# mahbhlddnhakkh/yuv-manipulations-2

Hardware: AMD Instinct MI355X
Metric: megapixels/sec DCT compress+decompress, 4K IYUV; achieved HBM GB/s vs peak (higher is better)
Workload: dtype u8/int16 (fp32 transform)

## Files before the change

yuv-manipulations-2_amd/csrc/fdct_bfly.h:

```cpp
#pragma once

#if defined(__HIPCC__)
#define MYYUV_BF_HD __host__ __device__ __forceinline__
#else
#include <math.h>
#define MYYUV_BF_HD static inline
#endif

namespace myyuv_bfly {

constexpr float kC0 = 0.3535533845424652f, kC4 = 0.3535534143447876f;
constexpr float kA2 = 0.4619397521018982f, kB2 = 0.19134166836738586f;
constexpr float kA6 = 0.4619397521018982f, kB6 = 0.19134169816970825f;
constexpr float kO1[4] = {0.49039262533187866f, 0.41573476791381836f, 0.27778512239456177f, 0.09754513204097748f};
constexpr float kO3[4] = {0.41573482751846313f, -0.0975450873374939f, -0.49039262533187866f, -0.277785062789917f};
constexpr float kO5[4] = {0.2777852416038513f, -0.49039262533187866f, 0.09754514694213867f, 0.41573476791381836f};
constexpr float kO7[4] = {0.09754543751478195f, -0.2777852416038513f, 0.4157347083091736f, -0.49039262533187866f};
constexpr float kBflyK = 7.946e-7f;

MYYUV_BF_HD float odd4(const float (&o)[4], float d0, float d1, float d2, float d3) {
  return fmaf(o[3], d3, fmaf(o[2], d2, fmaf(o[1], d1, o[0] * d0)));
}

MYYUV_BF_HD void bfly_cols(const float (&p)[8], float (&t)[8]) {
  const float s0 = p[0] + p[7], s1 = p[1] + p[6], s2 = p[2] + p[5], s3 = p[3] + p[4];
  const float d0 = p[0] - p[7], d1 = p[1] - p[6], d2 = p[2] - p[5], d3 = p[3] - p[4];
  const float ss0 = s0 + s3, ss1 = s1 + s2, ds0 = s0 - s3, ds1 = s1 - s2;
  t[0] = kC0 * ((ss0 + ss1) - 1024.0f);
  t[4] = kC4 * (ss0 - ss1);
  t[2] = fmaf(kA2, ds0, kB2 * ds1);
  t[6] = fmaf(kB6, ds0, -kA6 * ds1);
  t[1] = odd4(kO1, d0, d1, d2, d3);
  t[3] = odd4(kO3, d0, d1, d2, d3);
  t[5] = odd4(kO5, d0, d1, d2, d3);
  t[7] = odd4(kO7, d0, d1, d2, d3);
}

MYYUV_BF_HD void bfly_rows(const float (&x)[8], float (&y)[8]) {
  const float s0 = x[0] + x[7], s1 = x[1] + x[6], s2 = x[2] + x[5], s3 = x[3] + x[4];
  const float d0 = x[0] - x[7], d1 = x[1] - x[6], d2 = x[2] - x[5], d3 = x[3] - x[4];
  const float ss0 = s0 + s3, ss1 = s1 + s2, ds0 = s0 - s3, ds1 = s1 - s2;
  y[0] = kC0 * (ss0 + ss1);
  y[4] = kC4 * (ss0 - ss1);
  y[2] = fmaf(kA2, ds0, kB2 * ds1);
  y[6] = fmaf(kB6, ds0, -kA6 * ds1);
  y[1] = odd4(kO1, d0, d1, d2, d3);
  y[3] = odd4(kO3, d0, d1, d2, d3);
  y[5] = odd4(kO5, d0, d1, d2, d3);
  y[7] = odd4(kO7, d0, d1, d2, d3);
}

MYYUV_BF_HD void bfly_row_bounds(const float* r, float* kb) {
  for (int i = 0; i < 8; i++) {
    double m = 0.0;
    for (int v = 0; v < 8; v++) m = r[i * 8 + v] > m ? r[i * 8 + v] : m;
    kb[i] = (float)((double)kBflyK * m * (1.0 + 0x1p-20) * (1.0 + 0x1p-22));
  }
}

#if !defined(__HIPCC__)
static inline int bfly_block(const unsigned char* px, const float* R, const float* kb, short* out) {
  unsigned a = 0;
  for (int i = 0; i < 64; i++) a += px[i] > 128 ? px[i] - 128u : 128u - px[i];
  const float af = (float)a;
  float T[8][8];
  for (int k = 0; k < 8; k++) {
    float p[8], t[8];
    for (int m = 0; m < 8; m++) p[m] = (float)px[m * 8 + k];
    bfly_cols(p, t);
    for (int i = 0; i < 8; i++) T[i][k] = t[i];
  }
  int ok = 1;
  for (int i = 0; i < 8; i++) {
    float y[8];
    bfly_rows(T[i], y);
    float em = 0.0f;
    for (int v = 0; v < 8; v++) {
      const float t = y[v] * R[i * 8 + v];
      const float uu = t + 0x1.8p23f;
      const float e = t - (uu - 0x1.8p23f);
      em = fmaxf(em, fabsf(e));
      out[i * 8 + v] = (short)(int)(uu - 0x1.8p23f);
    }
    if (fmaf(af, kb[i], em) >= 0.5f) ok = 0;
// ... 7 lines not shown
```

yuv-manipulations-2_amd/csrc/k_transform.hip:

```cpp
#include <stddef.h>

#include "codec_common.hpp"
#include "xform_common.hpp"

#ifndef MYYUV_K1_OCC
#define MYYUV_K1_OCC 8
#endif
#define MYYUV_K1_ATTR __attribute__((amdgpu_waves_per_eu(MYYUV_K1_OCC, MYYUV_K1_OCC)))

namespace myyuv_gpu {

using namespace xf;

typedef unsigned short k1_us2 __attribute__((ext_vector_type(2)));

__device__ __forceinline__ void store_block_rows(const uint32_t (&c)[16], uint32_t q, uint32_t lane, bool live,
                                                 uint32_t g, uint4* dlo, uint4* dhi, uint8_t* __restrict__ rmask,
                                                 uint32_t* __restrict__ binfo, const uint4* zq,
                                                 uint4* __restrict__ sink) {
  uint4 lo, hi;
  uint32_t rm;
  pack_quads(c, q, lo, hi, rm);
  const uint4 z0 = zq[0], z1 = zq[1];
  const uint32_t wv[8] = {lo.x, lo.y, lo.z, lo.w, hi.x, hi.y, hi.z, hi.w};
  const uint32_t zv[8] = {z0.x, z0.y, z0.z, z0.w, z1.x, z1.y, z1.z, z1.w};
  k1_us2 cnt = {0, 0}, mx = {0, 0};
#pragma unroll
  for (int i = 0; i < 8; i++) {
    uint32_t fu, m16;
    asm("v_pk_min_u16 %0, %1, %2" : "=v"(fu) : "v"(wv[i]), "s"(0x00010001u));
    cnt += __builtin_bit_cast(k1_us2, fu);
    asm("v_pk_mul_lo_u16 %0, %1, %2" : "=v"(m16) : "v"(fu), "v"(zv[i]));
    mx = __builtin_elementwise_max(mx, __builtin_bit_cast(k1_us2, m16));
  }
  uint32_t nnz = (uint32_t)cnt.x + (uint32_t)cnt.y;
  uint32_t msz = mx.x > mx.y ? (uint32_t)mx.x : (uint32_t)mx.y;
#pragma unroll
  for (int d = 1; d < 4; d <<= 1) {
    const uint32_t o = d == 1 ? quad_xor1(nnz | (msz << 16)) : quad_xor2(nnz | (msz << 16));
    nnz += o & 0xFFFFu;
    msz = max(msz, o >> 16);
  }
  const bool nzl = (rm >> (2 * q)) & 1u, nzh = (rm >> (2 * q + 1)) & 1u;
  *(live ? rmask + g : reinterpret_cast<uint8_t*>(sink + 128) + lane) = (uint8_t)rm;
  const uint32_t dc = quad_lane0(lo.x);
  *(live ? binfo + g : reinterpret_cast<uint32_t*>(sink + 132) + lane) = binfo_word(rm, msz, class_of(nnz, msz), dc);
  *(nzl ? dlo : sink + lane) = lo;
  *(nzh ? dhi : sink + 64 + lane) = hi;
}

#ifndef MYYUV_K1_BUF
#define MYYUV_K1_BUF 1
#endif
typedef unsigned int k1_v4u __attribute__((ext_vector_type(4)));
constexpr uint32_t kOob = 0xFFFFFFFFu;

struct K1Rsrc {
  __amdgpu_buffer_rsrc_t coef, rmask, binfo;
};
__device__ __forceinline__ K1Rsrc k1_rsrc(uint4* coef, uint8_t* rmask, uint32_t* binfo, const FrameGeom& G) {
  const uint32_t nblk = G.cum[3] * G.nframes;
  K1Rsrc r;
  r.coef = __builtin_amdgcn_make_buffer_rsrc(coef, 0, (int)(((nblk + 63u) / 64u) * (kCoefQuadsPerWave * 16u)),
                                             0x00020000);
  r.rmask = __builtin_amdgcn_make_buffer_rsrc(rmask, 0, (int)nblk, 0x00020000);
  r.binfo = __builtin_amdgcn_make_buffer_rsrc(binfo, 0, (int)(nblk * 4u), 0x00020000);
  return r;
}

__device__ __forceinline__ void store_block_rows_buf(const uint32_t (&c)[16], uint32_t q, bool live, uint32_t g,
                                                     const K1Rsrc& R, const uint4* zq) {
  uint4 lo, hi;
  uint32_t rm;
  pack_quads(c, q, lo, hi, rm);
  const uint4 z0 = zq[0], z1 = zq[1];
  const uint32_t wv[8] = {lo.x, lo.y, lo.z, lo.w, hi.x, hi.y, hi.z, hi.w};
  const uint32_t zv[8] = {z0.x, z0.y, z0.z, z0.w, z1.x, z1.y, z1.z, z1.w};
  k1_us2 cnt = {0, 0}, mx = {0, 0};
#pragma unroll
  for (int i = 0; i < 8; i++) {
    uint32_t fu, m16;
    asm("v_pk_min_u16 %0, %1, %2" : "=v"(fu) : "v"(wv[i]), "s"(0x00010001u));
    cnt += __builtin_bit_cast(k1_us2, fu);
    asm("v_pk_mul_lo_u16 %0, %1, %2" : "=v"(m16) : "v"(fu), "v"(zv[i]));
    mx = __builtin_elementwise_max(mx, __builtin_bit_cast(k1_us2, m16));
  }
  uint32_t nnz = (uint32_t)cnt.x + (uint32_t)cnt.y;
  uint32_t msz = mx.x > mx.y ? (uint32_t)mx.x : (uint32_t)mx.y;
#pragma unroll
  for (int d = 1; d < 4; d <<= 1) {
    const uint32_t o = d == 1 ? quad_xor1(nnz | (msz << 16)) : quad_xor2(nnz | (msz << 16));
    nnz += o & 0xFFFFu;
    msz = max(msz, o >> 16);
  }
  const bool nzl = (rm >> (2 * q)) & 1u, nzh = (rm >> (2 * q + 1)) & 1u;
  const uint32_t dc = quad_lane0(lo.x);
  __builtin_amdgcn_raw_buffer_store_b8((uint8_t)rm, R.rmask, live ? g : kOob, 0, 0);
  __builtin_amdgcn_raw_buffer_store_b32(binfo_word(rm, msz, class_of(nnz, msz), dc), R.binfo, live ? 4u * g : kOob,
                                        0, 0);
  const uint32_t qo = coef_quad(g, 2 * q) * 16u;
  __builtin_amdgcn_raw_buffer_store_b128(k1_v4u{lo.x, lo.y, lo.z, lo.w}, R.coef, live && nzl ? qo : kOob, 0, 0);
  __builtin_amdgcn_raw_buffer_store_b128(k1_v4u{hi.x, hi.y, hi.z, hi.w}, R.coef, live && nzh ? qo + 1024u : kOob, 0,
                                         0);
}

__device__ __forceinline__ void stage_zz(uint4* szz) {
  if (threadIdx.x < 32) reinterpret_cast<uint32_t*>(szz)[threadIdx.x] = kZzPairs.v[threadIdx.x];
}


__global__ __launch_bounds__(256) MYYUV_K1_ATTR void k_fdct_quant(const uint8_t* __restrict__ frame, FrameGeom G,
                                                   const QTables* __restrict__ qt,
                                                   uint4* __restrict__ coef, uint8_t* __restrict__ rmask,
                                                   uint32_t* __restrict__ binfo, uint4* __restrict__ sink,
                                                   uint32_t* __restrict__ k2ctl, uint32_t* __restrict__ fix,
                                                   uint32_t par) {
  if (k2ctl != nullptr && blockIdx.x == 0 && threadIdx.x == 0) *k2ctl = 0u;
  __shared__ float tile[4][kXfUnit * kTile];
  __shared__ float sqr[kSqWords];
  __shared__ uint4 szz[8];
  static_assert(offsetof(QTables, r) == sizeof(float) * kSqR && offsetof(QTables, kb) == sizeof(float) * kSqKb,
                "layout");
  stage_zz(szz);
  stage_tables<kSqWords>(qt->q[0], sqr);
  if (kSinkSlots > 1) sink += (size_t)((blockIdx.x * 4u + (threadIdx.x >> 6)) % kSinkSlots) * kSinkQuads;
  const uint32_t lane = threadIdx.x & 63u;
  const uint32_t q = lane & 3u, b = lane >> 2;
  float* tb = tile[threadIdx.x >> 6] + b * kTile;
  uint8_t* img = reinterpret_cast<uint8_t*>(tb);
#if MYYUV_K1_BUF
  const K1Rsrc rs = k1_rsrc(coef, rmask, binfo, G);
#endif
  const uint32_t nall = G.ucum[3] * G.nframes, stride = unit_stride();
  uint32_t ua = first_unit();
  uint4 nx = ua < nall ? load_rows(frame, G, ua, b, q) : make_uint4(0, 0, 0, 0);
  sink[lane] = make_uint4(0, 0, 0, 0);
  sink[64 + lane] = make_uint4(0, 0, 0, 0);
  reinterpret_cast<uint8_t*>(sink + 128)[lane] = 0;

  for (; ua < nall; ua += stride) {
    const uint32_t f = div_magic(ua, G.umag);
    const Unit U = unit_of(G, ua - f * G.ucum[3]);
    const uint32_t local = U.local0 + b;
    const bool live = local < U.nb;
    const uint32_t g = f * G.cum[3] + U.cum + local;
    *reinterpret_cast<uint2*>(img + 16u * q) = make_uint2(nx.x, nx.y);
    *reinterpret_cast<uint2*>(img + 16u * q + 8u) = make_uint2(nx.z, nx.w);
    nx = load_rows(frame, G, ua + stride < nall ? ua + stride : ua, b, q);
    wave_sync();

    auto store = [&](const uint32_t (&c)[16], bool keep) {
      const bool lv = live && keep;
#if MYYUV_K1_BUF
      store_block_rows_buf(c, q, lv, g, rs, szz + 2 * q);
#else
      uint4* dlo = lv ? coef + coef_quad(g, 2 * q) : sink + lane;
      uint4* dhi = lv ? coef + coef_quad(g, 2 * q + 1) : sink + 64 + lane;
      store_block_rows(c, q, lane, lv, g, dlo, dhi, rmask, binfo, szz + 2 * q, sink);
#endif
    };
    uint32_t xr[4];
    fdct_load(img, q, xr);
    const uint64_t bad = fdct_fast<true>(xr, tb, q, sqr, U.p, store);
    if (bad != 0) {
      const bool mine = ((bad >> lane) & 1u) && q == 0 && live;
      const uint64_t m = __ballot(mine);
      const uint32_t c = ua % kFixLists;
      uint32_t base = 0;
      if (lane == 0 && m != 0) base = atomicAdd(fix_count(fix, par, c), (uint32_t)__popcll(m));
      base = __builtin_amdgcn_readfirstlane(base);
      const uint32_t idx = base + __builtin_amdgcn_mbcnt_hi((uint32_t)(m >> 32), __builtin_amdgcn_mbcnt_lo((uint32_t)m, 0u));
      if (mine && idx < fix_list_cap(nall)) fix_list(fix, G, c)[idx] = ua * kXfUnit + b;
    }
  }
}

__global__ __launch_bounds__(64 * kFixWaves) void k_fdct_fix(const uint8_t* __restrict__ frame, FrameGeom G,
                                                  const QTables* __restrict__ qt, uint4* __restrict__ coef,
                                                  uint8_t* __restrict__ rmask, uint32_t* __restrict__ binfo,
                                                  uint4* __restrict__ sink,
                                                  uint32_t* __restrict__ fix, uint32_t par) {
  __shared__ float tile[kFixWaves][kXfUnit * kTile];
  __shared__ float sqr[2 * 3 * 64];
  __shared__ uint4 szz[8];
  __shared__ uint32_t s_any;
  if (blockIdx.x == 0 && threadIdx.x < kFixLists) *fix_count(fix, par ^ 1u, threadIdx.x) = 0u;
  if (threadIdx.x == 0) s_any = 0u;
  __syncthreads();
  const uint32_t gw = blockIdx.x * kFixWaves + (threadIdx.x >> 6), nw = gridDim.x * kFixWaves;
  const uint32_t c = gw % kFixLists;
  const uint32_t n = __builtin_amdgcn_readfirstlane(*fix_count(fix, par, c));
  if ((threadIdx.x & 63u) == 0 && gw / kFixLists * kXfUnit < n) s_any = 1u;
  __syncthreads();
  if (s_any == 0u) return;
  stage_zz(szz);
#pragma unroll
  for (uint32_t i = threadIdx.x; i < 2u * 3u * 64u; i += 64u * kFixWaves) sqr[i] = qt->q[0][i];
  __syncthreads();
  const uint32_t lane = threadIdx.x & 63u;
  const uint32_t q = lane & 3u, b = lane >> 2;
  float* tb = tile[threadIdx.x >> 6] + b * kTile;
  uint8_t* img = reinterpret_cast<uint8_t*>(tb);
  const uint32_t* list = fix_list(fix, G, c);
#if MYYUV_K1_BUF
  const K1Rsrc rs = k1_rsrc(coef, rmask, binfo, G);
#endif
  for (uint32_t i = gw / kFixLists * kXfUnit; i < n; i += nw / kFixLists * kXfUnit) {
    const bool real = i + b < n;
    const uint32_t ent = list[real ? i + b : i];
    const uint32_t ua = ent / kXfUnit, bb = ent % kXfUnit;
    const uint32_t f = div_magic(ua, G.umag);
    const Unit U = unit_of(G, ua - f * G.ucum[3]);
    const uint32_t g = f * G.cum[3] + U.cum + U.local0 + bb;
    const uint4 r = load_rows(frame, G, ua, bb, q);
    wave_sync();
    *reinterpret_cast<uint2*>(img + 16u * q) = make_uint2(r.x, r.y);
    *reinterpret_cast<uint2*>(img + 16u * q + 8u) = make_uint2(r.z, r.w);
    wave_sync();
    uint32_t xr[4];
    fdct_load(img, q, xr);
#if MYYUV_K1_BUF
    fdct_exact(xr, tb, q, sqr, U.p, [&](const uint32_t (&cc)[16]) { store_block_rows_buf(cc, q, real, g, rs, szz + 2 * q); });
#else
    uint4* dlo = real ? coef + coef_quad(g, 2 * q) : sink + lane;
    uint4* dhi = real ? coef + coef_quad(g, 2 * q + 1) : sink + 64 + lane;
    fdct_exact(xr, tb, q, sqr, U.p,
               [&](const uint32_t (&cc)[16]) {
                 store_block_rows(cc, q, lane, real, g, dlo, dhi, rmask, binfo, szz + 2 * q, sink);
               });
#endif
  }
}

__global__ __launch_bounds__(256) void k_dequant_idct(const uint4* __restrict__ coef,
                                                     const uint8_t* __restrict__ rmask,
                                                     const uint4* __restrict__ zq, FrameGeom G,
                                                     const QTables* __restrict__ qt,
                                                     uint8_t* __restrict__ frame, uint4* __restrict__ sink) {
  __shared__ float tile[4][kXfUnit * kTile];
  __shared__ float sq[3 * 64];
  stage_tables<3 * 64>(qt->q[0], sq);
  const uint32_t lane = threadIdx.x & 63u;
  const uint32_t q = lane & 3u, b = lane >> 2;
// ... 102 lines not shown
```

yuv-manipulations-2_amd/csrc/myyuv_hip.cpp:

```cpp
#include <hip/hip_ext.h>
#include <hip/hip_runtime.h>

#include <algorithm>
#include <cmath>
#include <cstdio>
#include <cstdlib>
#include <cstring>
#include <mutex>
#include <vector>

#include "codec_common.hpp"
#include "fdct_bfly.h"
#include "k_chain.hpp"
#include "k_stream.hpp"
#include "myyuv_hip.h"

#ifndef MYYUV_R16_BATCH
#define MYYUV_R16_BATCH 1
#endif

namespace myyuv_gpu {
__global__ void k_fdct_quant(const uint8_t*, FrameGeom, const QTables*, uint4*, uint8_t*, uint32_t*, uint4*,
                             uint32_t*, uint32_t*, uint32_t);
__global__ void k_fdct_fix(const uint8_t*, FrameGeom, const QTables*, uint4*, uint8_t*, uint32_t*, uint4*,
// ... 1243 lines not shown
  std::vector<uint8_t> rm(n);
  if (hipStreamSynchronize(c->stream) != hipSuccess ||
      hipMemcpy(img.data(), c->coef.p, nq * 16, hipMemcpyDeviceToHost) != hipSuccess ||
      hipMemcpy(rm.data(), c->rmask.p, n, hipMemcpyDeviceToHost) != hipSuccess)
    return MYYUV_E_HIP;
  for (uint32_t b = 0; b < n; b++)
    for (uint32_t q = 0; q < 8; q++) {
      if ((rm[b] >> q) & 1u)
        std::memcpy(out + (size_t)b * 64 + q * 8, &img[coef_quad(b, q)], 16);
      else
        std::memset(out + (size_t)b * 64 + q * 8, 0, 16);
    }
  return 0;
}

int myyuv_debug_tinfo_guard(myyuv_hip_handle c, uint32_t ntiles, int arm, uint32_t* changed) {
  if (!c) return MYYUV_E_ARG;
  std::lock_guard<std::mutex> lk(c->mu);
  DeviceGuard g(c->device);
  constexpr uint32_t kGuardWords = kWinTilesBig * kTInfoWords;
  constexpr uint32_t kCanary = 0xA5C3E1F7u;
  const size_t off = (size_t)ntiles * kTInfoWords * 4;
  if (off + kGuardWords * 4 > c->tinfo.n) return MYYUV_E_ARG;
  std::vector<uint32_t> w(kGuardWords, kCanary);
  if (hipStreamSynchronize(c->stream) != hipSuccess) return MYYUV_E_HIP;
  uint8_t* p = static_cast<uint8_t*>(c->tinfo.p) + off;
  if (arm) return hipMemcpy(p, w.data(), kGuardWords * 4, hipMemcpyHostToDevice) == hipSuccess ? 0 : MYYUV_E_HIP;
  if (!changed) return MYYUV_E_ARG;
  if (hipMemcpy(w.data(), p, kGuardWords * 4, hipMemcpyDeviceToHost) != hipSuccess) return MYYUV_E_HIP;
  uint32_t n = 0;
// ... 116 lines not shown
```

yuv-manipulations-2_amd/csrc/xform_common.hpp:

```cpp
#pragma once
#include <stddef.h>

#include "codec_common.hpp"
#include "fdct_bfly.h"

namespace myyuv_gpu {
namespace xf {

constexpr float c_dct[64] = MYYUV_DCT_MATRIX;
constexpr int kTile = 72;
constexpr int kXfTile16 = 16 * kTile;
constexpr float kMagic = 0x1.8p23f;
constexpr float kMagicPx = 0x1.8p23f + 128.0f;
constexpr float kHalfDown = 0x1.fffffep-2f;

__device__ __forceinline__ constexpr int tix(int i, int j) { return (i >> 1) * 18 + 2 * j + (i & 1); }

__device__ __forceinline__ uint32_t bits(float x) { return __builtin_bit_cast(uint32_t, x); }

__device__ __forceinline__ void wave_sync() {
  __builtin_amdgcn_fence(__ATOMIC_RELEASE, "wavefront");
  __builtin_amdgcn_wave_barrier();
  __builtin_amdgcn_fence(__ATOMIC_ACQUIRE, "wavefront");
}
// ... 24 lines not shown
};

template <class T>
__device__ __forceinline__ T pick(bool p1, bool p2, T a0, T a1, T a2) {
  return p2 ? a2 : (p1 ? a1 : a0);
}

__device__ __forceinline__ Unit unit_of(const FrameGeom& G, uint32_t u) {
  const bool p1 = u >= G.ucum[1], p2 = u >= G.ucum[2];
  Unit r;
  r.p = p2 ? 2 : (p1 ? 1 : 0);
  r.local0 = (u - pick(p1, p2, G.ucum[0], G.ucum[1], G.ucum[2])) * kXfUnit;
  r.cum = pick(p1, p2, G.cum[0], G.cum[1], G.cum[2]);
  r.nb = pick(p1, p2, G.cum[1], G.cum[2], G.cum[3]) - r.cum;
  r.poff = pick(p1, p2, G.poff[0], G.poff[1], G.poff[2]);
  r.pw = pick(p1, p2, G.pw[0], G.pw[1], G.pw[2]);
  r.bw = pick(p1, p2, G.bw[0], G.bw[1], G.bw[2]);
  r.bmag = pick(p1, p2, G.bmag[0], G.bmag[1], G.bmag[2]);
  return r;
}

__device__ __forceinline__ uint32_t block_row_offset(const Unit& U, uint32_t local, uint32_t r) {
  uint32_t by = local;
  if (U.bmag != 0) {
    const uint64_t lo = (uint64_t)local * (uint32_t)U.bmag;
    const uint64_t hi = (uint64_t)local * (uint32_t)(U.bmag >> 32) + (lo >> 32);
    by = (uint32_t)(hi >> 32);
  }
  const uint32_t bx = local - by * U.bw;
  return U.poff + (by * 8u + r) * U.pw + bx * 8u;
}

__device__ __forceinline__ uint32_t first_unit() {
// ... 28 lines not shown
                                               float (&P)[16]) {
#pragma unroll
  for (int i = 0; i < 8; i++) {
    tb[tix(i, 2 * q)] = M[2 * i];
    tb[tix(i, 2 * q + 1)] = M[2 * i + 1];
  }
  wave_sync();
#pragma unroll
  for (int k = 0; k < 8; k++) {
    const float2 v = *reinterpret_cast<const float2*>(tb + tix(2 * q, k));
    P[2 * k] = v.x;
    P[2 * k + 1] = v.y;
  }
}

__device__ __forceinline__ float sbyte(uint32_t w, int k) {
  return (float)(int)(int8_t)(uint8_t)(w >> (8 * k));
}

__device__ __forceinline__ uint4 load_rows(const uint8_t* __restrict__ frame, const FrameGeom& G,
                                           uint32_t ua, uint32_t b, uint32_t q) {
  const uint32_t f = div_magic(ua, G.umag);
  const Unit U = unit_of(G, ua - f * G.ucum[3]);
  const uint32_t local = U.local0 + b;
  const uint32_t off = block_row_offset(U, local < U.nb ? local : U.nb - 1, 2u * q);
  const uint8_t* fr = frame + (size_t)f * G.fbytes;
  const uint2 r0 = *reinterpret_cast<const uint2*>(fr + off);
  const uint2 r1 = *reinterpret_cast<const uint2*>(fr + off + U.pw);
  return make_uint4(r0.x, r0.y, r1.x, r1.y);
}

template <int kWords>
// ... 9 lines not shown
  const uint32_t f = div_magic(ua, G.umag);
  const Unit U = unit_of(G, ua - f * G.ucum[3]);
  const uint32_t local = U.local0 + b;
  return f * G.cum[3] + U.cum + (local < U.nb ? local : U.nb - 1);
}

__device__ __forceinline__ void load_quads(const uint4* __restrict__ coef, const uint4* __restrict__ zq,
                                           uint32_t g, uint32_t q, uint32_t m, uint4& a, uint4& c) {
  const uint4* pa = (m >> (2 * q)) & 1u ? coef + coef_quad(g, 2 * q) : zq;
  const uint4* pc = (m >> (2 * q + 1)) & 1u ? coef + coef_quad(g, 2 * q + 1) : zq;
  a = *pa;
  c = *pc;
}


__device__ __forceinline__ void fdct_stage1_exact(const uint32_t (&xr)[4], float (&T)[16]) {
#pragma unroll
  for (int k = 0; k < 8; k++) {
    const uint32_t w = xr[k >> 1] ^ 0x80808080u;
    const float x0 = sbyte(w, 2 * (k & 1)), x1 = sbyte(w, 2 * (k & 1) + 1);
#pragma unroll
    for (int i = 0; i < 8; i++) {
      const float d = c_dct[i * 8 + k];
      const float p0 = d * x0, p1 = d * x1;
      T[2 * i] = k == 0 ? p0 : T[2 * i] + p0;
      T[2 * i + 1] = k == 0 ? p1 : T[2 * i + 1] + p1;
    }
    fence16(T);
  }
}


__device__ __forceinline__ void fdct_load(const uint8_t* img, uint32_t q, uint32_t (&xr)[4]) {
#pragma unroll
  for (int m = 0; m < 4; m++)
    xr[m] = *reinterpret_cast<const uint16_t*>(img + 16 * m + 2 * q) |
            ((uint32_t)*reinterpret_cast<const uint16_t*>(img + 16 * m + 8 + 2 * q) << 16);
  wave_sync();
}

constexpr int kSqR = 3 * 64, kSqKb = 2 * 3 * 64, kSqWords = 2 * 3 * 64 + 3 * 8;

template <bool kPerBlock, class Emit>
__device__ __forceinline__ uint64_t fdct_fast(const uint32_t (&xr)[4], float* tb, uint32_t q, const float* sqr, int p,
                                              Emit&& emit) {
  uint32_t a = 0;
#pragma unroll
  for (int m = 0; m < 4; m++) a = __builtin_amdgcn_sad_u8(xr[m], 0x80808080u, a);
  a += quad_xor1(a);
  a += quad_xor2(a);
  float T[16];
#pragma unroll
  for (int c = 0; c < 2; c++) {
    float px[8], t[8];
#pragma unroll
    for (int m = 0; m < 8; m++) px[m] = (float)((xr[m >> 1] >> (8 * (2 * (m & 1) + c))) & 0xFFu);
    myyuv_bfly::bfly_cols(px, t);
#pragma unroll
    for (int i = 0; i < 8; i++) T[2 * i + c] = t[i];
  }
  float P[16];
  transpose_tile(tb, q, T, P);
  const float af = (float)a;
  const float* Rq = sqr + kSqR + p * 64 + 16u * q;
  uint32_t c[16];
  float mx = 0.0f;
#pragma unroll
  for (int h = 0; h < 2; h++) {
    float x[8], y[8];
#pragma unroll
    for (int k = 0; k < 8; k++) x[k] = P[2 * k + h];
    myyuv_bfly::bfly_rows(x, y);
// ... 10 lines not shown
  }
  const uint64_t bad = __builtin_amdgcn_ballot_w64(mx >= 0.5f);
  if (bad == 0) {
    emit(c, true);
    return 0;
  }
  if (!kPerBlock) return bad;
  uint32_t fb = mx >= 0.5f ? 1u : 0u;
  fb |= quad_xor1(fb);
  fb |= quad_xor2(fb);
  emit(c, fb == 0u);
  return __builtin_amdgcn_ballot_w64(fb != 0u);
}

template <class Emit>
__device__ __forceinline__ void fdct_exact(const uint32_t (&xr)[4], float* tb, uint32_t q, const float* sqr, int p,
                                           Emit&& emit) {
  const uint32_t n0 = 16u * q;
  float T[16];
  fdct_stage1_exact(xr, T);
  float P[16];
  transpose_tile(tb, q, T, P);
  float Y[16];
  dot_rows<false>(P, Y);
  const float4* R4 = reinterpret_cast<const float4*>(sqr + kSqR + p * 64 + n0);
  const float4 r0 = R4[0], r1 = R4[1], r2 = R4[2], r3 = R4[3];
  const float rr[16] = {r0.x, r2.x, r0.y, r2.y, r0.z, r2.z, r0.w, r2.w,
                        r1.x, r3.x, r1.y, r3.y, r1.z, r3.z, r1.w, r3.w};
  uint32_t c[16];
  float mx = 0.0f;
#pragma unroll
  for (int j = 0; j < 16; j++) {
    const float tq = Y[j] * rr[j];
    const float uu = tq + kMagic;
    const float e = tq - (uu - kMagic);
    mx = __builtin_fmaxf(mx, __builtin_fmaf(__builtin_fabsf(tq), kNearRel, __builtin_fabsf(e)));
    c[j] = bits(uu);
  }
  if (mx >= 0.5f) {
    const float* Qt = sqr + p * 64 + n0;
#pragma unroll
    for (int j = 0; j < 16; j++) c[j] = (uint32_t)(int)roundf(Y[j] / Qt[(j >> 1) + 8 * (j & 1)]);
  }
  emit(c);
}

template <class Emit>
__device__ __forceinline__ void fdct_core(const uint8_t* img, float* tb, uint32_t q, const float* sqr, int p,
                                          Emit&& emit) {
  uint32_t xr[4];
  fdct_load(img, q, xr);
  if (__builtin_expect(fdct_fast<false>(xr, tb, q, sqr, p, emit) != 0, 0)) {
    wave_sync();
    fdct_exact(xr, tb, q, sqr, p, [&](const uint32_t (&c)[16]) { emit(c, true); });
  }
}

__device__ __forceinline__ void pack_quads(const uint32_t (&c)[16], uint32_t q, uint4& lo, uint4& hi,
                                           uint32_t& rm) {
  lo.x = __builtin_amdgcn_perm(c[2], c[0], 0x05040100u);
  lo.y = __builtin_amdgcn_perm(c[6], c[4], 0x05040100u);
  lo.z = __builtin_amdgcn_perm(c[10], c[8], 0x05040100u);
  lo.w = __builtin_amdgcn_perm(c[14], c[12], 0x05040100u);
  hi.x = __builtin_amdgcn_perm(c[3], c[1], 0x05040100u);
  hi.y = __builtin_amdgcn_perm(c[7], c[5], 0x05040100u);
  hi.z = __builtin_amdgcn_perm(c[11], c[9], 0x05040100u);
  hi.w = __builtin_amdgcn_perm(c[15], c[13], 0x05040100u);
  const bool nzl = (lo.x | lo.y | lo.z | lo.w) != 0u, nzh = (hi.x | hi.y | hi.z | hi.w) != 0u;
  rm = (nzl ? 1u << (2 * q) : 0u) | (nzh ? 2u << (2 * q) : 0u);
// ... 130 lines not shown
```

yuv-manipulations-2_amd/myyuv_hip.py:

```python
import ctypes
import os

import numpy as np

_HERE = os.path.dirname(os.path.abspath(__file__))
LIB_PATH = os.environ.get("MYYUV_HIP_LIB") or os.path.join(_HERE, "libmyyuv_hip.so")

OK = 0
E_ARG, E_QUALITY, E_WIDTH, E_HEIGHT, E_CAPACITY = 1, 2, 3, 4, 5
E_DCTYUV_SIZE, E_PLANE_SIZE, E_PLANE_NBLK, E_PLANE_CONTENT = 6, 7, 8, 9
E_BAD_CODE, E_UNKNOWN_SYMBOL, E_BAD_CHUNK, E_HIP, E_NO_DEVICE = 10, 11, 12, 13, 14
E_BMP_INVALID, E_BMP_SIGN, E_BMP_UNSUPPORTED = 15, 16, 17

KERNELS = ["fdct_quant", "huff_encode", "scan_tiles", "stream_out", "encode_tile", "huff_decode",
           "dequant_idct", "huff_encode_wide", "huff_encode_r16", "huff_encode_wave", "bmp_to_iyuv",
           "fdct_fix"]
(K_FDCT, K_HUFF_ENC, K_SCAN, K_COMPACT, K_ENCODE_TILE, K_HUFF_DEC, K_IDCT, K_HUFF_WIDE,
 K_HUFF_R16, K_HUFF_WAVE, K_BMP, K_FDCT_FIX) = range(len(KERNELS))

EXPORTS = [
    "myyuv_hip_create", "myyuv_hip_destroy", "myyuv_hip_strerror", "myyuv_dct_payload_bound",
    "myyuv_gpu_dct_compress", "myyuv_gpu_dct_decompress", "myyuv_hip_reserve",
    "myyuv_gpu_dct_compress_device", "myyuv_gpu_dct_decompress_device", "myyuv_hip_sync_status",
    "myyuv_hip_profile", "myyuv_hip_profile_kernels", "myyuv_hip_kernel_stats", "myyuv_gpu_fdct_blocks",
# ... 8 lines not shown


class CodecError(RuntimeError):

    def __init__(self, code, bad_block=-1):
        self.code = code
        self.bad_block = bad_block
        super().__init__(strerror(code) if _lib is not None else f"error {code}")


def _share_hip_runtime_with_torch():
    try:
        import torch
    except Exception:
        pass


def load():
    global _lib
    if _lib is not None:
        return _lib
    if os.environ.get("MYYUV_NO_TORCH_RUNTIME") != "1":
        _share_hip_runtime_with_torch()
    if not os.path.exists(LIB_PATH):
        raise FileNotFoundError(f"{LIB_PATH} missing: build it with `make -C yuv-manipulations-2_amd`"
                                " or __graft_entry__.build()")
    L = ctypes.CDLL(LIB_PATH)
    u8p = ctypes.POINTER(ctypes.c_uint8)
    vp = ctypes.c_void_p
    u32 = ctypes.c_uint32
# ... 272 lines not shown
    def kernel_stats(self):
        ms = (ctypes.c_double * len(KERNELS))()
        n = (ctypes.c_int64 * len(KERNELS))()
        rc = load().myyuv_hip_kernel_stats(self._h, ms, n)
        if rc:
            raise CodecError(rc)
        return {KERNELS[i]: (ms[i], n[i]) for i in range(len(KERNELS))}

    def tinfo_guard(self, ntiles, arm):
        n = ctypes.c_uint32(0)
        rc = load().myyuv_debug_tinfo_guard(self._h, int(ntiles), 1 if arm else 0, ctypes.byref(n))
        if rc:
            raise CodecError(rc)
        return n.value

    def fdct_blocks(self, px, qtable):
        px = np.ascontiguousarray(px, np.uint8).reshape(-1, 64)
        qt = np.ascontiguousarray(qtable, np.float32).reshape(64)
        out = np.empty((px.shape[0], 64), np.int16)
        rc = load().myyuv_gpu_fdct_blocks(self._h, _u8(px), px.shape[0],
                                          qt.ctypes.data_as(ctypes.POINTER(ctypes.c_float)),
                                          out.ctypes.data_as(ctypes.POINTER(ctypes.c_int16)))
        if rc:
            raise CodecError(rc)
        return out

    def huff_encode_blocks(self, coef_zz):
        c = np.ascontiguousarray(coef_zz, np.int16).reshape(-1, 64)
        n = c.shape[0]
        chunks = np.zeros((n, 160), np.uint8)
# ... 7 lines not shown
```

Baseline: 368,700.

## Use biased-float pixel loads and bitmask-based block stats in forward DCT kernel

Pixels are turned into floats by OR-ing the byte into the exponent pattern of 2^23 (biased float), which replaces integer unpack plus int-to-float conversions. The butterfly is rewritten to cancel the bias inside its sums and differences. Per-block nonzero count and max zig-zag index now come from a packed nonzero bitmask via popcount/clz and small LDS lookup tables, instead of packed-u16 multiply/max against a zig-zag table. Dead-lane stores use OR-ed out-of-bounds offsets instead of selects. This cuts ALU work in the transform kernel, at the cost of extra LDS tables and byte-wise LDS loads, and relies on subtle float-bias exactness.

```diff
diff --git a/yuv-manipulations-2_amd/csrc/fdct_bfly.h b/yuv-manipulations-2_amd/csrc/fdct_bfly.h
--- a/yuv-manipulations-2_amd/csrc/fdct_bfly.h
+++ b/yuv-manipulations-2_amd/csrc/fdct_bfly.h
@@ -4,6 +4,7 @@
 #define MYYUV_BF_HD __host__ __device__ __forceinline__
 #else
 #include <math.h>
+#include <string.h>
 #define MYYUV_BF_HD static inline
 #endif
 
@@ -22,9 +23,8 @@
   return fmaf(o[3], d3, fmaf(o[2], d2, fmaf(o[1], d1, o[0] * d0)));
 }
 
-MYYUV_BF_HD void bfly_cols(const float (&p)[8], float (&t)[8]) {
-  const float s0 = p[0] + p[7], s1 = p[1] + p[6], s2 = p[2] + p[5], s3 = p[3] + p[4];
-  const float d0 = p[0] - p[7], d1 = p[1] - p[6], d2 = p[2] - p[5], d3 = p[3] - p[4];
+MYYUV_BF_HD void bfly_cols_sd(float s0, float s1, float s2, float s3, float d0, float d1, float d2, float d3,
+                              float (&t)[8]) {
   const float ss0 = s0 + s3, ss1 = s1 + s2, ds0 = s0 - s3, ds1 = s1 - s2;
   t[0] = kC0 * ((ss0 + ss1) - 1024.0f);
   t[4] = kC4 * (ss0 - ss1);
@@ -34,6 +34,18 @@
   t[3] = odd4(kO3, d0, d1, d2, d3);
   t[5] = odd4(kO5, d0, d1, d2, d3);
   t[7] = odd4(kO7, d0, d1, d2, d3);
+}
+
+MYYUV_BF_HD void bfly_cols(const float (&p)[8], float (&t)[8]) {
+  bfly_cols_sd(p[0] + p[7], p[1] + p[6], p[2] + p[5], p[3] + p[4], p[0] - p[7], p[1] - p[6], p[2] - p[5],
+               p[3] - p[4], t);
+}
+
+constexpr unsigned kBiasBits = 0x4B000000u;
+constexpr float kBias2 = 16777216.0f;
+MYYUV_BF_HD void bfly_cols_biased(const float (&pb)[8], float (&t)[8]) {
+  bfly_cols_sd((pb[0] - kBias2) + pb[7], (pb[1] - kBias2) + pb[6], (pb[2] - kBias2) + pb[5],
+               (pb[3] - kBias2) + pb[4], pb[0] - pb[7], pb[1] - pb[6], pb[2] - pb[5], pb[3] - pb[4], t);
 }
 
 MYYUV_BF_HD void bfly_rows(const float (&x)[8], float (&y)[8]) {
@@ -59,6 +71,12 @@
 }
 
 #if !defined(__HIPCC__)
+static inline float biased_pixel(unsigned char x) {
+  const unsigned w = kBiasBits | x;
+  float f;
+  memcpy(&f, &w, sizeof f);
+  return f;
+}
 static inline int bfly_block(const unsigned char* px, const float* R, const float* kb, short* out) {
   unsigned a = 0;
   for (int i = 0; i < 64; i++) a += px[i] > 128 ? px[i] - 128u : 128u - px[i];
@@ -66,8 +84,8 @@
   float T[8][8];
   for (int k = 0; k < 8; k++) {
     float p[8], t[8];
-    for (int m = 0; m < 8; m++) p[m] = (float)px[m * 8 + k];
-    bfly_cols(p, t);
+    for (int m = 0; m < 8; m++) p[m] = biased_pixel(px[m * 8 + k]);
+    bfly_cols_biased(p, t);
     for (int i = 0; i < 8; i++) T[i][k] = t[i];
   }
   int ok = 1;
diff --git a/yuv-manipulations-2_amd/csrc/k_transform.hip b/yuv-manipulations-2_amd/csrc/k_transform.hip
--- a/yuv-manipulations-2_amd/csrc/k_transform.hip
+++ b/yuv-manipulations-2_amd/csrc/k_transform.hip
@@ -12,41 +12,97 @@
 
 using namespace xf;
 
-typedef unsigned short k1_us2 __attribute__((ext_vector_type(2)));
-
-__device__ __forceinline__ void store_block_rows(const uint32_t (&c)[16], uint32_t q, uint32_t lane, bool live,
-                                                 uint32_t g, uint4* dlo, uint4* dhi, uint8_t* __restrict__ rmask,
-                                                 uint32_t* __restrict__ binfo, const uint4* zq,
-                                                 uint4* __restrict__ sink) {
-  uint4 lo, hi;
-  uint32_t rm;
-  pack_quads(c, q, lo, hi, rm);
-  const uint4 z0 = zq[0], z1 = zq[1];
+
+struct K1Tables {
+  uint8_t last[72];
+  int8_t empty[72];
+  uint8_t cls[68];
+};
+struct ZzLast {
+  uint8_t v[72];
+  constexpr ZzLast() : v{} {
+    constexpr uint8_t zz[64] = MYYUV_ZIGZAG;
+    uint8_t inv[64] = {};
+    for (int i = 0; i < 64; i++) inv[zz[i]] = (uint8_t)(i + 1);
+    for (int r = 0; r < 8; r++)
+      for (int n = 1; n <= 8; n++) v[9 * r + n] = inv[r * 8 + n - 1];
+  }
+};
+constexpr ZzLast kZzLast{};
+constexpr bool zz_rows_increase() {
+  constexpr uint8_t zz[64] = MYYUV_ZIGZAG;
+  uint32_t inv[64] = {};
+  for (int i = 0; i < 64; i++) inv[zz[i]] = (uint32_t)i;
+  for (int n = 0; n < 64; n++)
+    if ((n & 7) != 0 && inv[n] <= inv[n - 1]) return false;
+  return true;
+}
+static_assert(zz_rows_increase(), "msz from the last nonzero column needs rows that increase in zig-zag order");
+
+__device__ __forceinline__ void stage_k1_tables(K1Tables& t) {
+  const uint32_t i = threadIdx.x;
+  if (i < 72) {
+    t.last[i] = kZzLast.v[i];
+    t.empty[i] = i % 9u != 0 ? 0 : ((i / 9u) & 1u ? -2 : -1);
+  }
+  if (i < 68) t.cls[i] = (uint8_t)class_of(i, i);
+}
+
+__device__ __forceinline__ uint32_t opaque(uint32_t v) {
+  asm("" : "+v"(v));
+  return v;
+}
+
+__device__ __forceinline__ void block_words(const uint32_t (&c)[16], uint32_t q, const K1Tables& tab,
+                                            const uint8_t* tl, uint4& lo, uint4& hi, uint32_t& rm, uint32_t& word,
+                                            uint32_t& el, uint32_t& eh) {
+  lo.x = __builtin_amdgcn_perm(c[2], c[0], 0x05040100u);
+  lo.y = __builtin_amdgcn_perm(c[6], c[4], 0x05040100u);
+  lo.z = __builtin_amdgcn_perm(c[10], c[8], 0x05040100u);
+  lo.w = __builtin_amdgcn_perm(c[14], c[12], 0x05040100u);
+  hi.x = __builtin_amdgcn_perm(c[3], c[1], 0x05040100u);
+  hi.y = __builtin_amdgcn_perm(c[7], c[5], 0x05040100u);
+  hi.z = __builtin_amdgcn_perm(c[11], c[9], 0x05040100u);
+  hi.w = __builtin_amdgcn_perm(c[15], c[13], 0x05040100u);
   const uint32_t wv[8] = {lo.x, lo.y, lo.z, lo.w, hi.x, hi.y, hi.z, hi.w};
-  const uint32_t zv[8] = {z0.x, z0.y, z0.z, z0.w, z1.x, z1.y, z1.z, z1.w};
-  k1_us2 cnt = {0, 0}, mx = {0, 0};
+  uint32_t m = 1u;
 #pragma unroll
   for (int i = 0; i < 8; i++) {
-    uint32_t fu, m16;
+    uint32_t fu;
     asm("v_pk_min_u16 %0, %1, %2" : "=v"(fu) : "v"(wv[i]), "s"(0x00010001u));
-    cnt += __builtin_bit_cast(k1_us2, fu);
-    asm("v_pk_mul_lo_u16 %0, %1, %2" : "=v"(m16) : "v"(fu), "v"(zv[i]));
-    mx = __builtin_elementwise_max(mx, __builtin_bit_cast(k1_us2, m16));
-  }
-  uint32_t nnz = (uint32_t)cnt.x + (uint32_t)cnt.y;
-  uint32_t msz = mx.x > mx.y ? (uint32_t)mx.x : (uint32_t)mx.y;
+    m |= fu << (2 * (i & 3) + 1 + 8 * (i >> 2));
+  }
+  const uint32_t z = opaque(m | (m >> 15)) & 0x1FFFFu;
+  uint32_t nnz = (uint32_t)__builtin_popcount(z) - 1u;
+  const uint32_t nl = 31u - (uint32_t)__builtin_clz(opaque(z & 0x1FFu) | 1u);
+  const uint32_t nh = 23u - (uint32_t)__builtin_clz(z | 0x100u);
+  uint32_t msz = max((uint32_t)tl[nl], (uint32_t)tl[9u + nh]);
+  el = (uint32_t)(int32_t)reinterpret_cast<const int8_t*>(tl)[offsetof(K1Tables, empty) + nl];
+  eh = (uint32_t)(int32_t)reinterpret_cast<const int8_t*>(tl)[offsetof(K1Tables, empty) + 9u + nh];
+  rm = (el + eh + 3u) << (2u * q);
+  rm |= quad_xor1(rm);
+  rm |= quad_xor2(rm);
 #pragma unroll
   for (int d = 1; d < 4; d <<= 1) {
     const uint32_t o = d == 1 ? quad_xor1(nnz | (msz << 16)) : quad_xor2(nnz | (msz << 16));
     nnz += o & 0xFFFFu;
     msz = max(msz, o >> 16);
   }
-  const bool nzl = (rm >> (2 * q)) & 1u, nzh = (rm >> (2 * q + 1)) & 1u;
+  const uint32_t cls = tab.cls[nnz + (opaque(nnz - msz) >> 31)];
+  word = binfo_word(rm, msz, cls, quad_lane0(lo.x));
+}
+
+__device__ __forceinline__ void store_block_rows(const uint32_t (&c)[16], uint32_t q, uint32_t lane, bool live,
+                                                 uint32_t g, uint4* dlo, uint4* dhi, uint8_t* __restrict__ rmask,
+                                                 uint32_t* __restrict__ binfo, const K1Tables& tab,
+                                                 const uint8_t* tl, uint4* __restrict__ sink) {
+  uint4 lo, hi;
+  uint32_t rm, word, el, eh;
+  block_words(c, q, tab, tl, lo, hi, rm, word, el, eh);
   *(live ? rmask + g : reinterpret_cast<uint8_t*>(sink + 128) + lane) = (uint8_t)rm;
-  const uint32_t dc = quad_lane0(lo.x);
-  *(live ? binfo + g : reinterpret_cast<uint32_t*>(sink + 132) + lane) = binfo_word(rm, msz, class_of(nnz, msz), dc);
-  *(nzl ? dlo : sink + lane) = lo;
-  *(nzh ? dhi : sink + 64 + lane) = hi;
+  *(live ? binfo + g : reinterpret_cast<uint32_t*>(sink + 132) + lane) = word;
+  *(el == 0 ? dlo : sink + lane) = lo;
+  *(eh == 0 ? dhi : sink + 64 + lane) = hi;
 }
 
 #ifndef MYYUV_K1_BUF
@@ -68,44 +124,17 @@
   return r;
 }
 
-__device__ __forceinline__ void store_block_rows_buf(const uint32_t (&c)[16], uint32_t q, bool live, uint32_t g,
-                                                     const K1Rsrc& R, const uint4* zq) {
+__device__ __forceinline__ void store_block_rows_buf(const uint32_t (&c)[16], uint32_t q, uint32_t dead, uint32_t g,
+                                                     const K1Rsrc& R, const K1Tables& tab, const uint8_t* tl) {
   uint4 lo, hi;
-  uint32_t rm;
-  pack_quads(c, q, lo, hi, rm);
-  const uint4 z0 = zq[0], z1 = zq[1];
-  const uint32_t wv[8] = {lo.x, lo.y, lo.z, lo.w, hi.x, hi.y, hi.z, hi.w};
-  const uint32_t zv[8] = {z0.x, z0.y, z0.z, z0.w, z1.x, z1.y, z1.z, z1.w};
-  k1_us2 cnt = {0, 0}, mx = {0, 0};
-#pragma unroll
-  for (int i = 0; i < 8; i++) {
-    uint32_t fu, m16;
-    asm("v_pk_min_u16 %0, %1, %2" : "=v"(fu) : "v"(wv[i]), "s"(0x00010001u));
-    cnt += __builtin_bit_cast(k1_us2, fu);
-    asm("v_pk_mul_lo_u16 %0, %1, %2" : "=v"(m16) : "v"(fu), "v"(zv[i]));
-    mx = __builtin_elementwise_max(mx, __builtin_bit_cast(k1_us2, m16));
-  }
-  uint32_t nnz = (uint32_t)cnt.x + (uint32_t)cnt.y;
-  uint32_t msz = mx.x > mx.y ? (uint32_t)mx.x : (uint32_t)mx.y;
-#pragma unroll
-  for (int d = 1; d < 4; d <<= 1) {
-    const uint32_t o = d == 1 ? quad_xor1(nnz | (msz << 16)) : quad_xor2(nnz | (msz << 16));
-    nnz += o & 0xFFFFu;
-    msz = max(msz, o >> 16);
-  }
-  const bool nzl = (rm >> (2 * q)) & 1u, nzh = (rm >> (2 * q + 1)) & 1u;
-  const uint32_t dc = quad_lane0(lo.x);
-  __builtin_amdgcn_raw_buffer_store_b8((uint8_t)rm, R.rmask, live ? g : kOob, 0, 0);
-  __builtin_amdgcn_raw_buffer_store_b32(binfo_word(rm, msz, class_of(nnz, msz), dc), R.binfo, live ? 4u * g : kOob,
-                                        0, 0);
+  uint32_t rm, word, el, eh;
+  block_words(c, q, tab, tl, lo, hi, rm, word, el, eh);
+  __builtin_amdgcn_raw_buffer_store_b8((uint8_t)rm, R.rmask, g | dead, 0, 0);
+  __builtin_amdgcn_raw_buffer_store_b32(word, R.binfo, (4u * g) | dead, 0, 0);
   const uint32_t qo = coef_quad(g, 2 * q) * 16u;
-  __builtin_amdgcn_raw_buffer_store_b128(k1_v4u{lo.x, lo.y, lo.z, lo.w}, R.coef, live && nzl ? qo : kOob, 0, 0);
-  __builtin_amdgcn_raw_buffer_store_b128(k1_v4u{hi.x, hi.y, hi.z, hi.w}, R.coef, live && nzh ? qo + 1024u : kOob, 0,
-                                         0);
-}
-
-__device__ __forceinline__ void stage_zz(uint4* szz) {
-  if (threadIdx.x < 32) reinterpret_cast<uint32_t*>(szz)[threadIdx.x] = kZzPairs.v[threadIdx.x];
+  const uint32_t qd = qo | dead;
+  __builtin_amdgcn_raw_buffer_store_b128(k1_v4u{lo.x, lo.y, lo.z, lo.w}, R.coef, qd | el, 0, 0);
+  __builtin_amdgcn_raw_buffer_store_b128(k1_v4u{hi.x, hi.y, hi.z, hi.w}, R.coef, opaque(qd | eh) | 1024u, 0, 0);
 }
 
 
@@ -118,16 +147,17 @@
   if (k2ctl != nullptr && blockIdx.x == 0 && threadIdx.x == 0) *k2ctl = 0u;
   __shared__ float tile[4][kXfUnit * kTile];
   __shared__ float sqr[kSqWords];
-  __shared__ uint4 szz[8];
+  __shared__ K1Tables stab;
   static_assert(offsetof(QTables, r) == sizeof(float) * kSqR && offsetof(QTables, kb) == sizeof(float) * kSqKb,
                 "layout");
-  stage_zz(szz);
+  stage_k1_tables(stab);
   stage_tables<kSqWords>(qt->q[0], sqr);
   if (kSinkSlots > 1) sink += (size_t)((blockIdx.x * 4u + (threadIdx.x >> 6)) % kSinkSlots) * kSinkQuads;
   const uint32_t lane = threadIdx.x & 63u;
   const uint32_t q = lane & 3u, b = lane >> 2;
   float* tb = tile[threadIdx.x >> 6] + b * kTile;
   uint8_t* img = reinterpret_cast<uint8_t*>(tb);
+  const uint8_t* tl = stab.last + 18u * q;
 #if MYYUV_K1_BUF
   const K1Rsrc rs = k1_rsrc(coef, rmask, binfo, G);
 #endif
@@ -142,28 +172,32 @@
     const uint32_t f = div_magic(ua, G.umag);
     const Unit U = unit_of(G, ua - f * G.ucum[3]);
     const uint32_t local = U.local0 + b;
-    const bool live = local < U.nb;
+    const uint32_t dead = (uint32_t)((int32_t)opaque(U.nb - 1u - local) >> 31);
+#if !MYYUV_K1_BUF
+    const bool live = dead == 0u;
+#endif
     const uint32_t g = f * G.cum[3] + U.cum + local;
     *reinterpret_cast<uint2*>(img + 16u * q) = make_uint2(nx.x, nx.y);
     *reinterpret_cast<uint2*>(img + 16u * q + 8u) = make_uint2(nx.z, nx.w);
+    const uint32_t a = sad128(nx);
     nx = load_rows(frame, G, ua + stride < nall ? ua + stride : ua, b, q);
     wave_sync();
 
     auto store = [&](const uint32_t (&c)[16], bool keep) {
+#if MYYUV_K1_BUF
+      store_block_rows_buf(c, q, keep ? dead : kOob, g, rs, stab, tl);
+#else
       const bool lv = live && keep;
-#if MYYUV_K1_BUF
-      store_block_rows_buf(c, q, lv, g, rs, szz + 2 * q);
-#else
       uint4* dlo = lv ? coef + coef_quad(g, 2 * q) : sink + lane;
       uint4* dhi = lv ? coef + coef_quad(g, 2 * q + 1) : sink + 64 + lane;
-      store_block_rows(c, q, lane, lv, g, dlo, dhi, rmask, binfo, szz + 2 * q, sink);
+      store_block_rows(c, q, lane, lv, g, dlo, dhi, rmask, binfo, stab, tl, sink);
 #endif
     };
-    uint32_t xr[4];
-    fdct_load(img, q, xr);
-    const uint64_t bad = fdct_fast<true>(xr, tb, q, sqr, U.p, store);
+    float pb[16];
+    fdct_load(img, q, pb);
+    const uint64_t bad = fdct_fast<true>(pb, a, tb, q, sqr, U.p, store);
     if (bad != 0) {
-      const bool mine = ((bad >> lane) & 1u) && q == 0 && live;
+      const bool mine = ((bad >> lane) & 1u) && q == 0 && dead == 0u;
       const uint64_t m = __ballot(mine);
       const uint32_t c = ua % kFixLists;
       uint32_t base = 0;
@@ -182,7 +216,7 @@
                                                   uint32_t* __restrict__ fix, uint32_t par) {
   __shared__ float tile[kFixWaves][kXfUnit * kTile];
   __shared__ float sqr[2 * 3 * 64];
-  __shared__ uint4 szz[8];
+  __shared__ K1Tables stab;
   __shared__ uint32_t s_any;
   if (blockIdx.x == 0 && threadIdx.x < kFixLists) *fix_count(fix, par ^ 1u, threadIdx.x) = 0u;
   if (threadIdx.x == 0) s_any = 0u;
@@ -193,7 +227,7 @@
   if ((threadIdx.x & 63u) == 0 && gw / kFixLists * kXfUnit < n) s_any = 1u;
   __syncthreads();
   if (s_any == 0u) return;
-  stage_zz(szz);
+  stage_k1_tables(stab);
 #pragma unroll
   for (uint32_t i = threadIdx.x; i < 2u * 3u * 64u; i += 64u * kFixWaves) sqr[i] = qt->q[0][i];
   __syncthreads();
@@ -201,6 +235,7 @@
   const uint32_t q = lane & 3u, b = lane >> 2;
   float* tb = tile[threadIdx.x >> 6] + b * kTile;
   uint8_t* img = reinterpret_cast<uint8_t*>(tb);
+  const uint8_t* tl = stab.last + 18u * q;
   const uint32_t* list = fix_list(fix, G, c);
 #if MYYUV_K1_BUF
   const K1Rsrc rs = k1_rsrc(coef, rmask, binfo, G);
@@ -217,16 +252,17 @@
     *reinterpret_cast<uint2*>(img + 16u * q) = make_uint2(r.x, r.y);
     *reinterpret_cast<uint2*>(img + 16u * q + 8u) = make_uint2(r.z, r.w);
     wave_sync();
-    uint32_t xr[4];
-    fdct_load(img, q, xr);
+    float pb[16];
+    fdct_load(img, q, pb);
 #if MYYUV_K1_BUF
-    fdct_exact(xr, tb, q, sqr, U.p, [&](const uint32_t (&cc)[16]) { store_block_rows_buf(cc, q, real, g, rs, szz + 2 * q); });
+    fdct_exact(pb, tb, q, sqr, U.p,
+               [&](const uint32_t (&cc)[16]) { store_block_rows_buf(cc, q, real ? 0u : kOob, g, rs, stab, tl); });
 #else
     uint4* dlo = real ? coef + coef_quad(g, 2 * q) : sink + lane;
     uint4* dhi = real ? coef + coef_quad(g, 2 * q + 1) : sink + 64 + lane;
-    fdct_exact(xr, tb, q, sqr, U.p,
+    fdct_exact(pb, tb, q, sqr, U.p,
                [&](const uint32_t (&cc)[16]) {
-                 store_block_rows(cc, q, lane, real, g, dlo, dhi, rmask, binfo, szz + 2 * q, sink);
+                 store_block_rows(cc, q, lane, real, g, dlo, dhi, rmask, binfo, stab, tl, sink);
                });
 #endif
   }
diff --git a/yuv-manipulations-2_amd/csrc/myyuv_hip.cpp b/yuv-manipulations-2_amd/csrc/myyuv_hip.cpp
--- a/yuv-manipulations-2_amd/csrc/myyuv_hip.cpp
+++ b/yuv-manipulations-2_amd/csrc/myyuv_hip.cpp
@@ -1281,6 +1281,20 @@
   return 0;
 }
 
+int myyuv_debug_block_words(myyuv_hip_handle c, uint32_t* binfo, uint8_t* rmask, uint32_t n) {
+  if (!c || !binfo || !rmask) return MYYUV_E_ARG;
+  std::lock_guard<std::mutex> lk(c->mu);
+  DeviceGuard g(c->device);
+  if ((size_t)n * 4 > c->binfo.n || n > c->rmask.n) return MYYUV_E_ARG;
+  if (hipStreamSynchronize(c->stream) != hipSuccess ||
+      hipMemcpy(binfo, c->binfo.p, (size_t)n * 4, hipMemcpyDeviceToHost) != hipSuccess ||
+      hipMemcpy(rmask, c->rmask.p, n, hipMemcpyDeviceToHost) != hipSuccess)
+    return MYYUV_E_HIP;
+  return 0;
+}
+
+uint32_t myyuv_debug_class_of(uint32_t nnz, uint32_t msz) { return class_of(nnz, msz); }
+
 int myyuv_debug_tinfo_guard(myyuv_hip_handle c, uint32_t ntiles, int arm, uint32_t* changed) {
   if (!c) return MYYUV_E_ARG;
   std::lock_guard<std::mutex> lk(c->mu);
diff --git a/yuv-manipulations-2_amd/csrc/xform_common.hpp b/yuv-manipulations-2_amd/csrc/xform_common.hpp
--- a/yuv-manipulations-2_amd/csrc/xform_common.hpp
+++ b/yuv-manipulations-2_amd/csrc/xform_common.hpp
@@ -62,9 +62,9 @@
   r.cum = pick(p1, p2, G.cum[0], G.cum[1], G.cum[2]);
   r.nb = pick(p1, p2, G.cum[1], G.cum[2], G.cum[3]) - r.cum;
   r.poff = pick(p1, p2, G.poff[0], G.poff[1], G.poff[2]);
-  r.pw = pick(p1, p2, G.pw[0], G.pw[1], G.pw[2]);
-  r.bw = pick(p1, p2, G.bw[0], G.bw[1], G.bw[2]);
-  r.bmag = pick(p1, p2, G.bmag[0], G.bmag[1], G.bmag[2]);
+  r.pw = p1 ? G.pw[1] : G.pw[0];
+  r.bw = p1 ? G.bw[1] : G.bw[0];
+  r.bmag = p1 ? G.bmag[1] : G.bmag[0];
   return r;
 }
 
@@ -123,8 +123,16 @@
   }
 }
 
-__device__ __forceinline__ float sbyte(uint32_t w, int k) {
-  return (float)(int)(int8_t)(uint8_t)(w >> (8 * k));
+__device__ __forceinline__ float biased(uint32_t x) {
+  return __builtin_bit_cast(float, myyuv_bfly::kBiasBits | x);
+}
+constexpr float kBias128 = 8388608.0f + 128.0f;
+
+__device__ __forceinline__ uint32_t sad128(const uint4& r) {
+  uint32_t a = __builtin_amdgcn_sad_u8(r.x, 0x80808080u, 0u);
+  a = __builtin_amdgcn_sad_u8(r.y, 0x80808080u, a);
+  a = __builtin_amdgcn_sad_u8(r.z, 0x80808080u, a);
+  return __builtin_amdgcn_sad_u8(r.w, 0x80808080u, a);
 }
 
 __device__ __forceinline__ uint4 load_rows(const uint8_t* __restrict__ frame, const FrameGeom& G,
@@ -164,11 +172,10 @@
 }
 
 
-__device__ __forceinline__ void fdct_stage1_exact(const uint32_t (&xr)[4], float (&T)[16]) {
-#pragma unroll
-  for (int k = 0; k < 8; k++) {
-    const uint32_t w = xr[k >> 1] ^ 0x80808080u;
-    const float x0 = sbyte(w, 2 * (k & 1)), x1 = sbyte(w, 2 * (k & 1) + 1);
+__device__ __forceinline__ void fdct_stage1_exact(const float (&pb)[16], float (&T)[16]) {
+#pragma unroll
+  for (int k = 0; k < 8; k++) {
+    const float x0 = pb[2 * k] - kBias128, x1 = pb[2 * k + 1] - kBias128;
 #pragma unroll
     for (int i = 0; i < 8; i++) {
       const float d = c_dct[i * 8 + k];
@@ -181,22 +188,25 @@
 }
 
 
-__device__ __forceinline__ void fdct_load(const uint8_t* img, uint32_t q, uint32_t (&xr)[4]) {
-#pragma unroll
-  for (int m = 0; m < 4; m++)
-    xr[m] = *reinterpret_cast<const uint16_t*>(img + 16 * m + 2 * q) |
-            ((uint32_t)*reinterpret_cast<const uint16_t*>(img + 16 * m + 8 + 2 * q) << 16);
+typedef const __attribute__((address_space(3))) uint8_t* lds_bytes;
+__device__ __forceinline__ void fdct_load(const uint8_t* img, uint32_t q, float (&pb)[16]) {
+  const lds_bytes c0 = (lds_bytes)(img + 2 * q);
+  uint32_t a1 = (uint32_t)(uintptr_t)c0 + 1u;
+  asm("" : "+v"(a1));
+  const lds_bytes c1 = (lds_bytes)(uintptr_t)a1;
+#pragma unroll
+  for (int m = 0; m < 8; m++) {
+    pb[2 * m] = biased(c0[8 * m]);
+    pb[2 * m + 1] = biased(c1[8 * m]);
+  }
   wave_sync();
 }
 
 constexpr int kSqR = 3 * 64, kSqKb = 2 * 3 * 64, kSqWords = 2 * 3 * 64 + 3 * 8;
 
 template <bool kPerBlock, class Emit>
-__device__ __forceinline__ uint64_t fdct_fast(const uint32_t (&xr)[4], float* tb, uint32_t q, const float* sqr, int p,
-                                              Emit&& emit) {
-  uint32_t a = 0;
-#pragma unroll
-  for (int m = 0; m < 4; m++) a = __builtin_amdgcn_sad_u8(xr[m], 0x80808080u, a);
+__device__ __forceinline__ uint64_t fdct_fast(const float (&pb)[16], uint32_t a, float* tb, uint32_t q,
+                                              const float* sqr, int p, Emit&& emit) {
   a += quad_xor1(a);
   a += quad_xor2(a);
   float T[16];
@@ -204,8 +214,8 @@
   for (int c = 0; c < 2; c++) {
     float px[8], t[8];
 #pragma unroll
-    for (int m = 0; m < 8; m++) px[m] = (float)((xr[m >> 1] >> (8 * (2 * (m & 1) + c))) & 0xFFu);
-    myyuv_bfly::bfly_cols(px, t);
+    for (int m = 0; m < 8; m++) px[m] = pb[2 * m + c];
+    myyuv_bfly::bfly_cols_biased(px, t);
 #pragma unroll
     for (int i = 0; i < 8; i++) T[2 * i + c] = t[i];
   }
@@ -246,11 +256,11 @@
 }
 
 template <class Emit>
-__device__ __forceinline__ void fdct_exact(const uint32_t (&xr)[4], float* tb, uint32_t q, const float* sqr, int p,
+__device__ __forceinline__ void fdct_exact(const float (&pb)[16], float* tb, uint32_t q, const float* sqr, int p,
                                            Emit&& emit) {
   const uint32_t n0 = 16u * q;
   float T[16];
-  fdct_stage1_exact(xr, T);
+  fdct_stage1_exact(pb, T);
   float P[16];
   transpose_tile(tb, q, T, P);
   float Y[16];
@@ -280,11 +290,12 @@
 template <class Emit>
 __device__ __forceinline__ void fdct_core(const uint8_t* img, float* tb, uint32_t q, const float* sqr, int p,
                                           Emit&& emit) {
-  uint32_t xr[4];
-  fdct_load(img, q, xr);
-  if (__builtin_expect(fdct_fast<false>(xr, tb, q, sqr, p, emit) != 0, 0)) {
+  const uint32_t a = sad128(*reinterpret_cast<const uint4*>(img + 16u * q));
+  float pb[16];
+  fdct_load(img, q, pb);
+  if (__builtin_expect(fdct_fast<false>(pb, a, tb, q, sqr, p, emit) != 0, 0)) {
     wave_sync();
-    fdct_exact(xr, tb, q, sqr, p, [&](const uint32_t (&c)[16]) { emit(c, true); });
+    fdct_exact(pb, tb, q, sqr, p, [&](const uint32_t (&c)[16]) { emit(c, true); });
   }
 }
 
diff --git a/yuv-manipulations-2_amd/myyuv_hip.py b/yuv-manipulations-2_amd/myyuv_hip.py
--- a/yuv-manipulations-2_amd/myyuv_hip.py
+++ b/yuv-manipulations-2_amd/myyuv_hip.py
@@ -46,6 +46,13 @@
         import torch
     except Exception:
         pass
+
+
+def class_of(nnz, msz):
+    f = load().myyuv_debug_class_of
+    f.argtypes = [ctypes.c_uint32, ctypes.c_uint32]
+    f.restype = ctypes.c_uint32
+    return int(f(int(nnz), int(msz)))
 
 
 def load():
@@ -348,6 +355,15 @@
             raise CodecError(rc)
         return n.value
 
+    def block_words(self, n):
+        binfo = np.empty(n, np.uint32)
+        rmask = np.empty(n, np.uint8)
+        rc = load().myyuv_debug_block_words(self._h, binfo.ctypes.data_as(ctypes.POINTER(ctypes.c_uint32)),
+                                            _u8(rmask), ctypes.c_uint32(n))
+        if rc:
+            raise CodecError(rc)
+        return binfo, rmask
+
     def fdct_blocks(self, px, qtable):
         px = np.ascontiguousarray(px, np.uint8).reshape(-1, 64)
         qt = np.ascontiguousarray(qtable, np.float32).reshape(64)
```

Result: no change. 366,200 (-0.7%).
